# larskaislaniemi/PyLamp

Hardware: AMD Instinct MI355X
Metric: stokes_heat_mic_cell_updates_per_s (higher is better)
Workload: dtype f64

## Files before the change

pylamp_amd/csrc/pl_mic_cells.hip:

```cpp
#include "pl_internal.h"
#include "pl_mic.h"

#define SC_Q 4
#define SC_NL 16
#define SC_W (SC_NL - 2)
#ifndef SC_ROWS
#define SC_ROWS 32
#endif
#ifndef SC_CAP
#define SC_CAP 320
#endif
#define SC_CAPP (SC_CAP + SC_CAP / 16 + 2)
#ifndef SC_NB
#define SC_NB 2
#endif

__device__ inline int sc_pidx(int o) { return o + (o >> 4); }

template <int CTRL> __device__ inline double sc_dpp(double v) {
    int lo = __double2loint(v), hi = __double2hiint(v);
    lo = __builtin_amdgcn_update_dpp(0, lo, CTRL, 0xf, 0xf, false);
    hi = __builtin_amdgcn_update_dpp(0, hi, CTRL, 0xf, 0xf, false);
    return __hiloint2double(hi, lo);
}
__device__ inline double sc_left(double v) { return sc_dpp<0x111>(v); }
__device__ inline double sc_right(double v) { return sc_dpp<0x101>(v); }
__device__ inline double sc_qsum(double v) {
    unsigned lo = (unsigned)__double2loint(v), hi = (unsigned)__double2hiint(v);
    auto rl = __builtin_amdgcn_permlane16_swap(lo, lo, false, false);
    auto rh = __builtin_amdgcn_permlane16_swap(hi, hi, false, false);
    v = __hiloint2double((int)rh[0], (int)rl[0]) + __hiloint2double((int)rh[1], (int)rl[1]);
    lo = (unsigned)__double2loint(v); hi = (unsigned)__double2hiint(v);
    rl = __builtin_amdgcn_permlane32_swap(lo, lo, false, false);
    rh = __builtin_amdgcn_permlane32_swap(hi, hi, false, false);
    return __hiloint2double((int)rh[0], (int)rl[0]) + __hiloint2double((int)rh[1], (int)rl[1]);
}

template <int NFN, int CEN, bool MID>
struct ScAcc {
    double N[2][2][1 + NFN];
    double C[CEN ? 3 : 1][CEN ? 3 : 1][2];
    double Z[MID ? 3 : 1][MID ? 2 : 1][2];
    double X[MID ? 2 : 1][MID ? 3 : 1][2];
};

template <bool FLAT>
__device__ inline void sc_slots3(double a, double w[3]) {
    const bool lo = a < 0.5;
    if (FLAT) { w[0] = lo ? 1.0 : 0.0; w[1] = 1.0; w[2] = lo ? 0.0 : 1.0; }
    else { w[0] = lo ? 0.5 - a : 0.0; w[1] = lo ? a + 0.5 : 1.5 - a; w[2] = lo ? 0.0 : a - 0.5; }
}

#define SC_IND_MASK ((1u << 2) | (1u << 4) | (1u << 5))
template <int NFN, int CEN, bool MID, bool IND>
__global__ __launch_bounds__(64) void k_scatter_cells(PlScatterCellsArgs a, int strips_x) {
    constexpr int NST = 2 + NFN + (MID ? 1 : 0);
    constexpr unsigned IMASK = IND ? SC_IND_MASK : 0u;
    __shared__ double lds[NST][SC_CAPP];
    __shared__ int csl[SC_ROWS + 2][SC_NL + 1];
    const int lane = threadIdx.x, q = lane >> 4, L = lane & 15;
    const int sx = blockIdx.x % strips_x, sy = blockIdx.x / strips_x;
    const int c0 = sx * SC_W, r0 = sy * SC_ROWS, r1 = min(r0 + SC_ROWS, a.ncz);
    const int cc = c0 + L - 1;
    const bool real = cc >= 0 && cc < a.ncx;
    const int gj = a.ccol0 + cc;
    const int nown = min(SC_W, a.ncx - c0);
    const bool last_x = c0 + SC_W >= a.ncx, last_z = r1 >= a.ncz;
    const bool col_own = ((L >= 1 && L <= nown) || (sx == 0 && L == 0) || (last_x && L == nown + 1)) && gj >= 0 && gj < a.nx &&
                         gj >= a.col0 && gj < a.col0 + a.ncols;
    const int R0 = a.crow0 + (sy == 0 ? r0 - 1 : r0), R1 = a.crow0 + (last_z ? r1 + 1 : r1);
    const int i0 = max(r0 - 1, 0), i1 = min(r1 + 1, a.ncz);
    const int cfirst = max(c0 - 1, 0), clast = min(c0 + SC_W + 1, a.ncx);
    for (int k = lane; k < (i1 - i0) * (SC_NL + 1); k += 64) {
        const int r = k / (SC_NL + 1), c = k % (SC_NL + 1);
        const int col = min(max(c0 - 1 + c, cfirst), clast);
        csl[r][c] = a.cell_start[(long long)(i0 + r) * a.ncx + col];
    }
    const double xc = a.x0 + gj * a.hx;
    __shared__ double car[NFN + 11][SC_NL];
    double* const cN = &car[0][L];
    double* const cX = &car[NFN + 1][L]; double* const qZ = &car[NFN + 3][L]; double* const pZ = &car[NFN + 5][L];
    double* const qC = &car[NFN + 7][L]; double* const pC = &car[NFN + 9][L];
    if (q == 0)
        for (int k = 0; k < NFN + 11; k++) car[k][L] = 0.0;
    auto emit = [&](double* plane, int gi_row, double v) {
        if (!col_own || gi_row < R0 || gi_row >= R1 || gi_row < 0 || gi_row >= a.nz || gi_row < a.row0 || gi_row >= a.row0 + a.nrows) return;
        plane[(long long)(gi_row - a.row0) * a.ncols + (gj - a.col0)] = v;
    };
    __syncthreads();
    constexpr int NU = SC_CAP / 64;
    double pf[NU][NST];
    __shared__ int ixs[IND ? SC_CAP : 1];
    int pix[NU];
    auto prefetch = [&](int row) {
        const int b0 = csl[row - i0][0], b1 = min(b0 + SC_CAP, csl[row - i0][SC_NL]);
#pragma unroll
        for (int u = 0; u < NU; u++) {
            const int t = b0 + lane + 64 * u;
            if (t < b1) {
                pf[u][0] = a.tz[t]; pf[u][1] = a.tx[t];
                const int e = IND ? ixs[lane + 64 * u] : t;
#pragma unroll
                for (int k = 0; k < NFN; k++) pf[u][2 + k] = a.fn[k][(IMASK >> k) & 1u ? e : t];
                if (MID) pf[u][2 + NFN] = a.fm[IND ? e : t];
            }
        }
        if (IND && row + 1 < i1) {
            const int c0n = csl[row + 1 - i0][0], c1n = min(c0n + SC_CAP, csl[row + 1 - i0][SC_NL]);
#pragma unroll
            for (int u = 0; u < NU; u++) { const int t = c0n + lane + 64 * u; if (t < c1n) pix[u] = a.ix[t]; }
        }
    };
    if (i0 < i1 && !(a.dbg & 8)) {
        if (IND) {
            const int b0 = csl[0][0], b1 = min(b0 + SC_CAP, csl[0][SC_NL]);
#pragma unroll
            for (int u = 0; u < NU; u++) { const int t = b0 + lane + 64 * u; if (t < b1) ixs[lane + 64 * u] = a.ix[t]; }
            __syncthreads();
        }
        prefetch(i0);
    }
    for (int i = i0; i < i1; i++) {
        const int gi = a.crow0 + i;
        const double zc = a.z0 + gi * a.hz;
        const int wrow0 = csl[i - i0][0], wrow1 = csl[i - i0][SC_NL];
        int s = 0, e = 0;
        if (real) { s = csl[i - i0][L]; e = csl[i - i0][L + 1]; }
        ScAcc<NFN, CEN, MID> A;
#pragma unroll
        for (int di = 0; di < 2; di++)
#pragma unroll
            for (int dj = 0; dj < 2; dj++)
#pragma unroll
                for (int k = 0; k <= NFN; k++) A.N[di][dj][k] = 0.0;
        if (CEN) {
#pragma unroll
            for (int u = 0; u < 3; u++)
#pragma unroll
                for (int v = 0; v < 3; v++) { A.C[u][v][0] = 0.0; A.C[u][v][1] = 0.0; }
        }
        if (MID) {
#pragma unroll
            for (int u = 0; u < 3; u++)
#pragma unroll
                for (int v = 0; v < 2; v++) { A.Z[u][v][0] = 0.0; A.Z[u][v][1] = 0.0; A.X[v][u][0] = 0.0; A.X[v][u][1] = 0.0; }
        }
        if (!(a.dbg & 8)) {
            const int we0 = min(wrow0 + SC_CAP, wrow1);
#pragma unroll
            for (int u = 0; u < NU; u++) {
                const int t = wrow0 + lane + 64 * u;
                if (t < we0) {
                    const int o = sc_pidx(t - wrow0);
#pragma unroll
                    for (int k = 0; k < NST; k++) lds[k][o] = pf[u][k];
                }
            }
            if (IND && i + 1 < i1) {
                const int c0n = csl[i + 1 - i0][0], c1n = min(c0n + SC_CAP, csl[i + 1 - i0][SC_NL]);
#pragma unroll
                for (int u = 0; u < NU; u++) if (c0n + lane + 64 * u < c1n) ixs[lane + 64 * u] = pix[u];
            }
        }
        __syncthreads();
        if (i + 1 < i1 && !(a.dbg & 8)) prefetch(i + 1);
        for (int wb = wrow0; wb < wrow1; wb += SC_CAP) {
            const int we = min(wb + SC_CAP, wrow1);
            if (wb != wrow0) {
                __syncthreads();
                constexpr int UB = (NU + SC_NB - 1) / SC_NB;
#pragma unroll
                for (int b = 0; b < SC_NB; b++) {
                    double st[UB][NST];
#pragma unroll
                    for (int u = 0; u < UB; u++) {
                        const int t = wb + lane + 64 * (b * UB + u);
                        if (b * UB + u < NU && t < we) {
                            st[u][0] = a.tz[t]; st[u][1] = a.tx[t];
                            const int e = IND ? a.ix[t] : t;
#pragma unroll
                            for (int k = 0; k < NFN; k++) st[u][2 + k] = a.fn[k][(IMASK >> k) & 1u ? e : t];
                            if (MID) st[u][2 + NFN] = a.fm[IND ? e : t];
                        }
                    }
#pragma unroll
                    for (int u = 0; u < UB; u++) {
                        const int t = wb + lane + 64 * (b * UB + u);
                        if (b * UB + u < NU && t < we) {
                            const int o = sc_pidx(t - wb);
#pragma unroll
                            for (int k = 0; k < NST; k++) lds[k][o] = st[u][k];
                        }
                    }
                }
                __syncthreads();
            }
            int t = s + q;
            if (t < wb) t += ((wb - t + SC_Q - 1) / SC_Q) * SC_Q;
            const int tend = min(e, we);
            for (; t < tend && !(a.dbg & 1); t += SC_Q) {
                const int o = sc_pidx(t - wb);
                const double z = lds[0][o], x = lds[1][o];
                const double ca = (z - zc) * a.rhz, cb = (x - xc) * a.rhx;
                if (!(ca >= 0.0 && ca < 1.0 && cb >= 0.0 && cb < 1.0)) {
                    if (L >= 1 && L <= nown && i >= r0 && i < r1) {
                        const int k = atomicAdd(a.slow_count, 1);
                        if (k < a.slow_cap) a.slow_list[k] = t;
                    }
                    continue;
                }
                double f[NFN > 0 ? NFN : 1];
#pragma unroll
                for (int k = 0; k < NFN; k++) f[k] = lds[2 + k][o];
                const double wz2[2] = {1.0 - ca, ca}, wx2[2] = {1.0 - cb, cb};
#pragma unroll
                for (int di = 0; di < 2; di++)
#pragma unroll
                    for (int dj = 0; dj < 2; dj++) {
                        const double w = wx2[dj] * wz2[di];
                        A.N[di][dj][0] += w;
#pragma unroll
                        for (int k = 0; k < NFN; k++) A.N[di][dj][1 + k] += f[k] * w;
                    }
                double wz3[3], wx3[3];
                if (CEN || MID) { sc_slots3<CEN == 2>(ca, wz3); sc_slots3<CEN == 2>(cb, wx3); }
                if (CEN) {
                    const double fc = f[NFN > 1 ? 1 : 0];
#pragma unroll
                    for (int u = 0; u < 3; u++)
#pragma unroll
                        for (int v = 0; v < 3; v++) {
                            const double w = wx3[v] * wz3[u];
                            A.C[u][v][0] += w; A.C[u][v][1] += fc * w;
                        }
                }
                if (MID) {
                    const double fm = lds[2 + NFN][o];
#pragma unroll
                    for (int u = 0; u < 3; u++)
#pragma unroll
                        for (int v = 0; v < 2; v++) {
                            const double wzm = wx2[v] * wz3[u];
                            A.Z[u][v][0] += wzm; A.Z[u][v][1] += fm * wzm;
                            const double wxm = wx3[u] * wz2[v];
                            A.X[v][u][0] += wxm; A.X[v][u][1] += fm * wxm;
                        }
                }
            }
        }
        double Hn[2][1 + NFN], Hz[3][2], Hx[2][2], Hc[3][2];
#pragma unroll
        for (int di = 0; di < 2; di++)
#pragma unroll
            for (int k = 0; k <= NFN; k++) Hn[di][k] = sc_qsum(A.N[di][0][k] + sc_left(A.N[di][1][k]));
        if (MID) {
#pragma unroll
            for (int u = 0; u < 3; u++)
#pragma unroll
                for (int k = 0; k < 2; k++) Hz[u][k] = sc_qsum(A.Z[u][0][k] + sc_left(A.Z[u][1][k]));
#pragma unroll
            for (int v = 0; v < 2; v++)
#pragma unroll
                for (int k = 0; k < 2; k++) Hx[v][k] = sc_qsum(A.X[v][1][k] + sc_left(A.X[v][2][k]) + sc_right(A.X[v][0][k]));
        }
        if (CEN) {
#pragma unroll
            for (int u = 0; u < 3; u++)
#pragma unroll
                for (int k = 0; k < 2; k++) Hc[u][k] = sc_qsum(A.C[u][1][k] + sc_left(A.C[u][2][k]) + sc_right(A.C[u][0][k]));
        }
        if (q == 0 && !(a.dbg & 4)) {
#pragma unroll
            for (int k = 0; k <= NFN; k++) {
                emit(a.accN + (long long)k * a.N, gi, Hn[0][k] + cN[k * SC_NL]);
                cN[k * SC_NL] = Hn[1][k];
            }
            if (MID) {
#pragma unroll
                for (int k = 0; k < 2; k++) {
                    emit(a.accX + (long long)k * a.N, gi, Hx[0][k] + cX[k * SC_NL]);
                    cX[k * SC_NL] = Hx[1][k];
                    emit(a.accZ + (long long)k * a.N, gi - 1, qZ[k * SC_NL] + Hz[0][k]);
                    qZ[k * SC_NL] = Hz[1][k] + pZ[k * SC_NL]; pZ[k * SC_NL] = Hz[2][k];
                }
            }
            if (CEN) {
#pragma unroll
                for (int k = 0; k < 2; k++) {
                    emit(a.accC + (long long)k * a.N, gi - 1, qC[k * SC_NL] + Hc[0][k]);
                    qC[k * SC_NL] = Hc[1][k] + pC[k * SC_NL]; pC[k * SC_NL] = Hc[2][k];
                }
            }
        }
        __syncthreads();
    }
    if (q == 0 && i1 > i0 && !(a.dbg & 4)) {
        const int gl = a.crow0 + i1;
#pragma unroll
        for (int k = 0; k <= NFN; k++) emit(a.accN + (long long)k * a.N, gl, cN[k * SC_NL]);
        if (MID) {
#pragma unroll
            for (int k = 0; k < 2; k++) {
                emit(a.accX + (long long)k * a.N, gl, cX[k * SC_NL]);
                emit(a.accZ + (long long)k * a.N, gl - 1, qZ[k * SC_NL]);
                emit(a.accZ + (long long)k * a.N, gl, pZ[k * SC_NL]);
            }
        }
        if (CEN) {
#pragma unroll
            for (int k = 0; k < 2; k++) {
                emit(a.accC + (long long)k * a.N, gl - 1, qC[k * SC_NL]);
                emit(a.accC + (long long)k * a.N, gl, pC[k * SC_NL]);
            }
        }
    }
}

template <int NFN, int CEN, bool MID, bool IND>
__global__ __launch_bounds__(256) void k_scatter_cells_slow(PlScatterCellsArgs a) {
    constexpr unsigned IMASK = IND ? SC_IND_MASK : 0u;
    const int n = min(*a.slow_count, a.slow_cap);
    for (int k = blockIdx.x * 256 + threadIdx.x; k < n; k += gridDim.x * 256) {
        const int t = a.slow_list[k];
        const int e = IND ? a.ix[t] : t;
        const double z = a.tz[t], x = a.tx[t];
        auto add = [&](double* plane, int ni, int nj, double v) {
            if (ni < 0 || ni >= a.nz || nj < 0 || nj >= a.nx || ni < a.row0 || ni >= a.row0 + a.nrows || nj < a.col0 || nj >= a.col0 + a.ncols) return;
            unsafeAtomicAdd(plane + (long long)(ni - a.row0) * a.ncols + (nj - a.col0), v);
        };
        for (int set = 0; set < 4; set++) {
            if ((set == 1 && !CEN) || (set >= 2 && !MID)) continue;
            const bool sz = set == 1 || set == 2, sx = set == 1 || set == 3;
            const double zo = a.z0 + (sz ? 0.5 * a.hz : 0.0), xo = a.x0 + (sx ? 0.5 * a.hx : 0.0);
            const double fz = floor((z - zo) * a.rhz), fx = floor((x - xo) * a.rhx);
            const int ie = (int)fz, je = (int)fx;
            const double ca = (z - (zo + fz * a.hz)) * a.rhz, cb = (x - (xo + fx * a.hx)) * a.rhx;
            double* base = set == 0 ? a.accN : set == 1 ? a.accC : set == 2 ? a.accZ : a.accX;
            const int nfs = set == 0 ? NFN : 1;
            for (int cnr = 0; cnr < 4; cnr++) {
                const int di = cnr & 1, dj = cnr >> 1;
                double w = (dj ? cb : 1.0 - cb) * (di ? ca : 1.0 - ca);
                const bool flat = set == 1 && CEN == 2;
                if (flat) w = 1.0;
                add(base, ie + di, je + dj, w);
                for (int f = 0; f < nfs; f++) {
                    const int fk = set == 0 ? f : (NFN > 1 ? 1 : 0);
                    const double v = set <= 1 ? a.fn[fk][(IMASK >> fk) & 1u ? e : t] : a.fm[IND ? e : t];
                    add(base + (long long)(1 + f) * a.N, ie + di, je + dj, v * w);
                }
            }
        }
    }
}

__global__ __launch_bounds__(256) void k_scatter_finalize_multi(PlScatterFinalArgs a) {
    const int j = blockIdx.x * 64 + threadIdx.x, i = blockIdx.y * 4 + threadIdx.y;
    if (j >= a.nx || i >= a.nz) return;
    const long long o = (long long)i * a.acc_pitch + j, oo = a.out_off + (long long)i * a.out_pitch + j;
    for (int k = 0; k < a.nf; k++) {
        double s = a.acc[k][o];
        const double d = a.den[k][o];
        double r;
        if (a.scheme[k] & PL_AVG_ARITHMETIC) r = s / d;
        else { if (isinf(s)) s = 0.0; r = exp(s / d); }
        a.out[k][oo] = r;
    }
}

void pl_launch_scatter_finalize_multi(pl_ctx* ctx, const PlScatterFinalArgs& a) {
    if (a.nf <= 0) return;
    hipLaunchKernelGGL(k_scatter_finalize_multi, dim3((a.nx + 63) / 64, (a.nz + 3) / 4), dim3(64, 4), 0, ctx->stream, a);
}

template <int NFN, int CEN, bool MID, bool IND = false>
static void launch_cells(pl_ctx* ctx, const PlScatterCellsArgs& a) {
    const int strips_x = (a.ncx + SC_W - 1) / SC_W, strips_z = (a.ncz + SC_ROWS - 1) / SC_ROWS;
    hipLaunchKernelGGL((k_scatter_cells<NFN, CEN, MID, IND>), dim3((unsigned)(strips_x * strips_z)), dim3(64), 0, ctx->stream, a, strips_x);
    hipLaunchKernelGGL((k_scatter_cells_slow<NFN, CEN, MID, IND>), dim3(32), dim3(256), 0, ctx->stream, a);
}

int pl_scatter_cells_device(pl_ctx* ctx, PlScatterCellsArgs& a, int variant) {
    if (a.ncz <= 0 || a.ncx <= 0) return 0;
    a.rhz = 1.0 / a.hz; a.rhx = 1.0 / a.hx;
    PL_HIP(ctx, hipMemsetAsync(a.slow_count, 0, sizeof(int), ctx->stream));
    if (a.ix && (variant != 0 || a.ind != (SC_IND_MASK | (1u << 31)))) return pl_fail(ctx, "pl_scatter_cells_device: unsupported set of indexed fields");
    if (variant == 0 && a.ix) launch_cells<6, 1, true, true>(ctx, a);
    else if (variant == 0) launch_cells<6, 1, true>(ctx, a);
    else if (variant == 1) launch_cells<2, 2, false>(ctx, a);
    else if (variant == 2) launch_cells<1, 0, false>(ctx, a);
    else return pl_fail(ctx, "pl_scatter_cells_device: unknown variant");
    PL_HIP(ctx, hipGetLastError());
    return 0;
}
```

Baseline: 203.3 million.

## Split scatter accumulator sets across waves and add deterministic listed slow path

The per-strip marker-to-grid scatter kernel now runs several wavefronts per block, each owning a subset of the accumulator sets (nodal, centre, z-mid, x-mid). The wavefronts share the staged LDS marker data and split the prefetch/copy work. This lowers per-wave register pressure and raises parallelism per strip, at the cost of redundant weight computation and larger blocks. A new single-block kernel handles up to 2048 out-of-cell markers without atomics, using a rank sort and row-banded serial accumulation. It is launched every call, even when there are no such markers, which adds launch latency.

Measured after the change: 206.3 million (median of 6 runs). 1.01x the previous value.

```diff
diff --git a/pylamp_amd/csrc/pl_mic_cells.hip b/pylamp_amd/csrc/pl_mic_cells.hip
--- a/pylamp_amd/csrc/pl_mic_cells.hip
+++ b/pylamp_amd/csrc/pl_mic_cells.hip
@@ -36,12 +36,25 @@
     return __hiloint2double((int)rh[0], (int)rl[0]) + __hiloint2double((int)rh[1], (int)rl[1]);
 }
 
-template <int NFN, int CEN, bool MID>
+#define SC_SET_N 1u
+#define SC_SET_C 2u
+#define SC_SET_Z 4u
+#define SC_SET_X 8u
+constexpr int sc_split_nw(int split) { return split == 1 ? 4 : split == 2 ? 3 : split == 3 ? 2 : 1; }
+constexpr unsigned sc_split_sets(int split, int w) {
+    return split == 1 ? (1u << w) : split == 2 ? (w == 0 ? SC_SET_N : w == 1 ? SC_SET_C : (SC_SET_Z | SC_SET_X))
+         : split == 3 ? (w == 0 ? SC_SET_N : (SC_SET_C | SC_SET_Z | SC_SET_X)) : (SC_SET_N | SC_SET_C | SC_SET_Z | SC_SET_X);
+}
+#ifndef SC_SPLIT_HEAT
+#define SC_SPLIT_HEAT 2
+#endif
+
+template <int NFN, bool SN, int CEN, bool SZ, bool SX>
 struct ScAcc {
-    double N[2][2][1 + NFN];
+    double N[SN ? 2 : 1][SN ? 2 : 1][SN ? 1 + NFN : 1];
     double C[CEN ? 3 : 1][CEN ? 3 : 1][2];
-    double Z[MID ? 3 : 1][MID ? 2 : 1][2];
-    double X[MID ? 2 : 1][MID ? 3 : 1][2];
+    double Z[SZ ? 3 : 1][SZ ? 2 : 1][2];
+    double X[SX ? 2 : 1][SX ? 3 : 1][2];
 };
 
 template <bool FLAT>
@@ -52,13 +65,15 @@
 }
 
 #define SC_IND_MASK ((1u << 2) | (1u << 4) | (1u << 5))
-template <int NFN, int CEN, bool MID, bool IND>
-__global__ __launch_bounds__(64) void k_scatter_cells(PlScatterCellsArgs a, int strips_x) {
+template <int NFN, int CEN, bool MID, bool IND, int NW, unsigned SETS>
+__device__ __forceinline__ void sc_strip(const PlScatterCellsArgs a, int strips_x, double (&lds)[2 + NFN + (MID ? 1 : 0)][SC_CAPP],
+                                         int (&csl)[SC_ROWS + 2][SC_NL + 1], double (&car)[NFN + 11][SC_NL], int (&ixs)[IND ? SC_CAP : 1]) {
     constexpr int NST = 2 + NFN + (MID ? 1 : 0);
     constexpr unsigned IMASK = IND ? SC_IND_MASK : 0u;
-    __shared__ double lds[NST][SC_CAPP];
-    __shared__ int csl[SC_ROWS + 2][SC_NL + 1];
-    const int lane = threadIdx.x, q = lane >> 4, L = lane & 15;
+    constexpr int NT = 64 * NW;
+    constexpr bool SN = (SETS & SC_SET_N) != 0, SC = (SETS & SC_SET_C) != 0 && CEN != 0, SZ = (SETS & SC_SET_Z) != 0 && MID,
+                   SX = (SETS & SC_SET_X) != 0 && MID;
+    const int tid = threadIdx.x, lane = tid & 63, q = lane >> 4, L = lane & 15;
     const int sx = blockIdx.x % strips_x, sy = blockIdx.x / strips_x;
     const int c0 = sx * SC_W, r0 = sy * SC_ROWS, r1 = min(r0 + SC_ROWS, a.ncz);
     const int cc = c0 + L - 1;
@@ -71,35 +86,33 @@
     const int R0 = a.crow0 + (sy == 0 ? r0 - 1 : r0), R1 = a.crow0 + (last_z ? r1 + 1 : r1);
     const int i0 = max(r0 - 1, 0), i1 = min(r1 + 1, a.ncz);
     const int cfirst = max(c0 - 1, 0), clast = min(c0 + SC_W + 1, a.ncx);
-    for (int k = lane; k < (i1 - i0) * (SC_NL + 1); k += 64) {
+    for (int k = tid; k < (i1 - i0) * (SC_NL + 1); k += NT) {
         const int r = k / (SC_NL + 1), c = k % (SC_NL + 1);
         const int col = min(max(c0 - 1 + c, cfirst), clast);
         csl[r][c] = a.cell_start[(long long)(i0 + r) * a.ncx + col];
     }
     const double xc = a.x0 + gj * a.hx;
-    __shared__ double car[NFN + 11][SC_NL];
     double* const cN = &car[0][L];
     double* const cX = &car[NFN + 1][L]; double* const qZ = &car[NFN + 3][L]; double* const pZ = &car[NFN + 5][L];
     double* const qC = &car[NFN + 7][L]; double* const pC = &car[NFN + 9][L];
-    if (q == 0)
+    if (tid < SC_NL)
         for (int k = 0; k < NFN + 11; k++) car[k][L] = 0.0;
     auto emit = [&](double* plane, int gi_row, double v) {
         if (!col_own || gi_row < R0 || gi_row >= R1 || gi_row < 0 || gi_row >= a.nz || gi_row < a.row0 || gi_row >= a.row0 + a.nrows) return;
         plane[(long long)(gi_row - a.row0) * a.ncols + (gj - a.col0)] = v;
     };
     __syncthreads();
-    constexpr int NU = SC_CAP / 64;
+    constexpr int NU = (SC_CAP + NT - 1) / NT;
     double pf[NU][NST];
-    __shared__ int ixs[IND ? SC_CAP : 1];
     int pix[NU];
     auto prefetch = [&](int row) {
         const int b0 = csl[row - i0][0], b1 = min(b0 + SC_CAP, csl[row - i0][SC_NL]);
 #pragma unroll
         for (int u = 0; u < NU; u++) {
-            const int t = b0 + lane + 64 * u;
+            const int t = b0 + tid + NT * u;
             if (t < b1) {
                 pf[u][0] = a.tz[t]; pf[u][1] = a.tx[t];
-                const int e = IND ? ixs[lane + 64 * u] : t;
+                const int e = IND ? ixs[tid + NT * u] : t;
 #pragma unroll
                 for (int k = 0; k < NFN; k++) pf[u][2 + k] = a.fn[k][(IMASK >> k) & 1u ? e : t];
                 if (MID) pf[u][2 + NFN] = a.fm[IND ? e : t];
@@ -108,14 +121,14 @@
         if (IND && row + 1 < i1) {
             const int c0n = csl[row + 1 - i0][0], c1n = min(c0n + SC_CAP, csl[row + 1 - i0][SC_NL]);
 #pragma unroll
-            for (int u = 0; u < NU; u++) { const int t = c0n + lane + 64 * u; if (t < c1n) pix[u] = a.ix[t]; }
+            for (int u = 0; u < NU; u++) { const int t = c0n + tid + NT * u; if (t < c1n) pix[u] = a.ix[t]; }
         }
     };
     if (i0 < i1 && !(a.dbg & 8)) {
         if (IND) {
             const int b0 = csl[0][0], b1 = min(b0 + SC_CAP, csl[0][SC_NL]);
 #pragma unroll
-            for (int u = 0; u < NU; u++) { const int t = b0 + lane + 64 * u; if (t < b1) ixs[lane + 64 * u] = a.ix[t]; }
+            for (int u = 0; u < NU; u++) { const int t = b0 + tid + NT * u; if (t < b1) ixs[tid + NT * u] = a.ix[t]; }
             __syncthreads();
         }
         prefetch(i0);
@@ -126,30 +139,33 @@
         const int wrow0 = csl[i - i0][0], wrow1 = csl[i - i0][SC_NL];
         int s = 0, e = 0;
         if (real) { s = csl[i - i0][L]; e = csl[i - i0][L + 1]; }
-        ScAcc<NFN, CEN, MID> A;
-#pragma unroll
-        for (int di = 0; di < 2; di++)
-#pragma unroll
-            for (int dj = 0; dj < 2; dj++)
-#pragma unroll
-                for (int k = 0; k <= NFN; k++) A.N[di][dj][k] = 0.0;
-        if (CEN) {
+        ScAcc<NFN, SN, SC ? CEN : 0, SZ, SX> A;
+        if constexpr (SN) {
+#pragma unroll
+            for (int di = 0; di < 2; di++)
+#pragma unroll
+                for (int dj = 0; dj < 2; dj++)
+#pragma unroll
+                    for (int k = 0; k <= NFN; k++) A.N[di][dj][k] = 0.0;
+        }
+        if constexpr (SC) {
 #pragma unroll
             for (int u = 0; u < 3; u++)
 #pragma unroll
                 for (int v = 0; v < 3; v++) { A.C[u][v][0] = 0.0; A.C[u][v][1] = 0.0; }
         }
-        if (MID) {
-#pragma unroll
-            for (int u = 0; u < 3; u++)
-#pragma unroll
-                for (int v = 0; v < 2; v++) { A.Z[u][v][0] = 0.0; A.Z[u][v][1] = 0.0; A.X[v][u][0] = 0.0; A.X[v][u][1] = 0.0; }
-        }
+#pragma unroll
+        for (int u = 0; u < 3; u++)
+#pragma unroll
+            for (int v = 0; v < 2; v++) {
+                if constexpr (SZ) { A.Z[u][v][0] = 0.0; A.Z[u][v][1] = 0.0; }
+                if constexpr (SX) { A.X[v][u][0] = 0.0; A.X[v][u][1] = 0.0; }
+            }
         if (!(a.dbg & 8)) {
             const int we0 = min(wrow0 + SC_CAP, wrow1);
 #pragma unroll
             for (int u = 0; u < NU; u++) {
-                const int t = wrow0 + lane + 64 * u;
+                const int t = wrow0 + tid + NT * u;
                 if (t < we0) {
                     const int o = sc_pidx(t - wrow0);
 #pragma unroll
@@ -159,7 +175,7 @@
             if (IND && i + 1 < i1) {
                 const int c0n = csl[i + 1 - i0][0], c1n = min(c0n + SC_CAP, csl[i + 1 - i0][SC_NL]);
 #pragma unroll
-                for (int u = 0; u < NU; u++) if (c0n + lane + 64 * u < c1n) ixs[lane + 64 * u] = pix[u];
+                for (int u = 0; u < NU; u++) if (c0n + tid + NT * u < c1n) ixs[tid + NT * u] = pix[u];
             }
         }
         __syncthreads();
@@ -174,18 +190,18 @@
                     double st[UB][NST];
 #pragma unroll
                     for (int u = 0; u < UB; u++) {
-                        const int t = wb + lane + 64 * (b * UB + u);
+                        const int t = wb + tid + NT * (b * UB + u);
                         if (b * UB + u < NU && t < we) {
                             st[u][0] = a.tz[t]; st[u][1] = a.tx[t];
                             const int e = IND ? a.ix[t] : t;
 #pragma unroll
                             for (int k = 0; k < NFN; k++) st[u][2 + k] = a.fn[k][(IMASK >> k) & 1u ? e : t];
-                            if (MID) st[u][2 + NFN] = a.fm[IND ? e : t];
+                            if constexpr (MID) st[u][2 + NFN] = a.fm[IND ? e : t];
                         }
                     }
 #pragma unroll
                     for (int u = 0; u < UB; u++) {
-                        const int t = wb + lane + 64 * (b * UB + u);
+                        const int t = wb + tid + NT * (b * UB + u);
                         if (b * UB + u < NU && t < we) {
                             const int o = sc_pidx(t - wb);
 #pragma unroll
@@ -203,29 +219,31 @@
                 const double z = lds[0][o], x = lds[1][o];
                 const double ca = (z - zc) * a.rhz, cb = (x - xc) * a.rhx;
                 if (!(ca >= 0.0 && ca < 1.0 && cb >= 0.0 && cb < 1.0)) {
-                    if (L >= 1 && L <= nown && i >= r0 && i < r1) {
+                    if (SN && L >= 1 && L <= nown && i >= r0 && i < r1) {
                         const int k = atomicAdd(a.slow_count, 1);
                         if (k < a.slow_cap) a.slow_list[k] = t;
                     }
                     continue;
                 }
+                const double wz2[2] = {1.0 - ca, ca}, wx2[2] = {1.0 - cb, cb};
                 double f[NFN > 0 ? NFN : 1];
-#pragma unroll
-                for (int k = 0; k < NFN; k++) f[k] = lds[2 + k][o];
-                const double wz2[2] = {1.0 - ca, ca}, wx2[2] = {1.0 - cb, cb};
-#pragma unroll
-                for (int di = 0; di < 2; di++)
-#pragma unroll
-                    for (int dj = 0; dj < 2; dj++) {
-                        const double w = wx2[dj] * wz2[di];
-                        A.N[di][dj][0] += w;
-#pragma unroll
-                        for (int k = 0; k < NFN; k++) A.N[di][dj][1 + k] += f[k] * w;
-                    }
+                if constexpr (SN) {
+#pragma unroll
+                    for (int k = 0; k < NFN; k++) f[k] = lds[2 + k][o];
+#pragma unroll
+                    for (int di = 0; di < 2; di++)
+#pragma unroll
+                        for (int dj = 0; dj < 2; dj++) {
+                            const double w = wx2[dj] * wz2[di];
+                            A.N[di][dj][0] += w;
+#pragma unroll
+                            for (int k = 0; k < NFN; k++) A.N[di][dj][1 + k] += f[k] * w;
+                        }
+                }
                 double wz3[3], wx3[3];
-                if (CEN || MID) { sc_slots3<CEN == 2>(ca, wz3); sc_slots3<CEN == 2>(cb, wx3); }
-                if (CEN) {
-                    const double fc = f[NFN > 1 ? 1 : 0];
+                if constexpr (SC || SZ || SX) { sc_slots3<CEN == 2>(ca, wz3); sc_slots3<CEN == 2>(cb, wx3); }
+                if constexpr (SC) {
+                    const double fc = SN ? f[NFN > 1 ? 1 : 0] : lds[2 + (NFN > 1 ? 1 : 0)][o];
 #pragma unroll
                     for (int u = 0; u < 3; u++)
 #pragma unroll
@@ -234,57 +252,69 @@
                             A.C[u][v][0] += w; A.C[u][v][1] += fc * w;
                         }
                 }
-                if (MID) {
+                if constexpr (SZ || SX) {
                     const double fm = lds[2 + NFN][o];
 #pragma unroll
                     for (int u = 0; u < 3; u++)
 #pragma unroll
                         for (int v = 0; v < 2; v++) {
-                            const double wzm = wx2[v] * wz3[u];
-                            A.Z[u][v][0] += wzm; A.Z[u][v][1] += fm * wzm;
-                            const double wxm = wx3[u] * wz2[v];
-                            A.X[v][u][0] += wxm; A.X[v][u][1] += fm * wxm;
+                            if constexpr (SZ) {
+                                const double wzm = wx2[v] * wz3[u];
+                                A.Z[u][v][0] += wzm; A.Z[u][v][1] += fm * wzm;
+                            }
+                            if constexpr (SX) {
+                                const double wxm = wx3[u] * wz2[v];
+                                A.X[v][u][0] += wxm; A.X[v][u][1] += fm * wxm;
+                            }
                         }
                 }
             }
         }
         double Hn[2][1 + NFN], Hz[3][2], Hx[2][2], Hc[3][2];
-#pragma unroll
-        for (int di = 0; di < 2; di++)
-#pragma unroll
-            for (int k = 0; k <= NFN; k++) Hn[di][k] = sc_qsum(A.N[di][0][k] + sc_left(A.N[di][1][k]));
-        if (MID) {
+        if constexpr (SN) {
+#pragma unroll
+            for (int di = 0; di < 2; di++)
+#pragma unroll
+                for (int k = 0; k <= NFN; k++) Hn[di][k] = sc_qsum(A.N[di][0][k] + sc_left(A.N[di][1][k]));
+        }
+        if constexpr (SZ) {
 #pragma unroll
             for (int u = 0; u < 3; u++)
 #pragma unroll
                 for (int k = 0; k < 2; k++) Hz[u][k] = sc_qsum(A.Z[u][0][k] + sc_left(A.Z[u][1][k]));
+        }
+        if constexpr (SX) {
 #pragma unroll
             for (int v = 0; v < 2; v++)
 #pragma unroll
                 for (int k = 0; k < 2; k++) Hx[v][k] = sc_qsum(A.X[v][1][k] + sc_left(A.X[v][2][k]) + sc_right(A.X[v][0][k]));
         }
-        if (CEN) {
+        if constexpr (SC) {
 #pragma unroll
             for (int u = 0; u < 3; u++)
 #pragma unroll
                 for (int k = 0; k < 2; k++) Hc[u][k] = sc_qsum(A.C[u][1][k] + sc_left(A.C[u][2][k]) + sc_right(A.C[u][0][k]));
         }
         if (q == 0 && !(a.dbg & 4)) {
-#pragma unroll
-            for (int k = 0; k <= NFN; k++) {
-                emit(a.accN + (long long)k * a.N, gi, Hn[0][k] + cN[k * SC_NL]);
-                cN[k * SC_NL] = Hn[1][k];
-            }
-            if (MID) {
-#pragma unroll
-                for (int k = 0; k < 2; k++) {
+            if constexpr (SN) {
+#pragma unroll
+                for (int k = 0; k <= NFN; k++) {
+                    emit(a.accN + (long long)k * a.N, gi, Hn[0][k] + cN[k * SC_NL]);
+                    cN[k * SC_NL] = Hn[1][k];
+                }
+            }
+#pragma unroll
+            for (int k = 0; k < 2; k++) {
+                if constexpr (SX) {
                     emit(a.accX + (long long)k * a.N, gi, Hx[0][k] + cX[k * SC_NL]);
                     cX[k * SC_NL] = Hx[1][k];
+                }
+                if constexpr (SZ) {
                     emit(a.accZ + (long long)k * a.N, gi - 1, qZ[k * SC_NL] + Hz[0][k]);
                     qZ[k * SC_NL] = Hz[1][k] + pZ[k * SC_NL]; pZ[k * SC_NL] = Hz[2][k];
                 }
             }
-            if (CEN) {
+            if constexpr (SC) {
 #pragma unroll
                 for (int k = 0; k < 2; k++) {
                     emit(a.accC + (long long)k * a.N, gi - 1, qC[k * SC_NL] + Hc[0][k]);
@@ -296,22 +326,96 @@
     }
     if (q == 0 && i1 > i0 && !(a.dbg & 4)) {
         const int gl = a.crow0 + i1;
-#pragma unroll
-        for (int k = 0; k <= NFN; k++) emit(a.accN + (long long)k * a.N, gl, cN[k * SC_NL]);
-        if (MID) {
-#pragma unroll
-            for (int k = 0; k < 2; k++) {
-                emit(a.accX + (long long)k * a.N, gl, cX[k * SC_NL]);
+        if constexpr (SN) {
+#pragma unroll
+            for (int k = 0; k <= NFN; k++) emit(a.accN + (long long)k * a.N, gl, cN[k * SC_NL]);
+        }
+#pragma unroll
+        for (int k = 0; k < 2; k++) {
+            if constexpr (SX) emit(a.accX + (long long)k * a.N, gl, cX[k * SC_NL]);
+            if constexpr (SZ) {
                 emit(a.accZ + (long long)k * a.N, gl - 1, qZ[k * SC_NL]);
                 emit(a.accZ + (long long)k * a.N, gl, pZ[k * SC_NL]);
             }
         }
-        if (CEN) {
+        if constexpr (SC) {
 #pragma unroll
             for (int k = 0; k < 2; k++) {
                 emit(a.accC + (long long)k * a.N, gl - 1, qC[k * SC_NL]);
                 emit(a.accC + (long long)k * a.N, gl, pC[k * SC_NL]);
             }
+        }
+    }
+}
+
+template <int NFN, int CEN, bool MID, bool IND, int SPLIT>
+__global__ __launch_bounds__(64 * sc_split_nw(SPLIT)) void k_scatter_cells(PlScatterCellsArgs a, int strips_x) {
+    constexpr int NW = sc_split_nw(SPLIT);
+    __shared__ double lds[2 + NFN + (MID ? 1 : 0)][SC_CAPP];
+    __shared__ int csl[SC_ROWS + 2][SC_NL + 1];
+    __shared__ double car[NFN + 11][SC_NL];
+    __shared__ int ixs[IND ? SC_CAP : 1];
+    const int wv = NW > 1 ? __builtin_amdgcn_readfirstlane((int)threadIdx.x >> 6) : 0;
+    if (wv == 0) sc_strip<NFN, CEN, MID, IND, NW, sc_split_sets(SPLIT, 0)>(a, strips_x, lds, csl, car, ixs);
+    if constexpr (NW > 1) { if (wv == 1) sc_strip<NFN, CEN, MID, IND, NW, sc_split_sets(SPLIT, 1)>(a, strips_x, lds, csl, car, ixs); }
+    if constexpr (NW > 2) { if (wv == 2) sc_strip<NFN, CEN, MID, IND, NW, sc_split_sets(SPLIT, 2)>(a, strips_x, lds, csl, car, ixs); }
+    if constexpr (NW > 3) { if (wv == 3) sc_strip<NFN, CEN, MID, IND, NW, sc_split_sets(SPLIT, 3)>(a, strips_x, lds, csl, car, ixs); }
+}
+
+#define SC_SLOW_DET 2048
+#define SC_SLOW_BANDS 64
+template <int NFN, int CEN, bool MID, bool IND>
+__global__ __launch_bounds__(1024) void k_scatter_cells_listed(PlScatterCellsArgs a) {
+    constexpr unsigned IMASK = IND ? SC_IND_MASK : 0u;
+    constexpr int NPL = (1 + NFN) + (CEN ? 2 : 0) + (MID ? 4 : 0);
+    static_assert(NPL * SC_SLOW_BANDS <= 1024, "one thread per plane and band");
+    __shared__ int raw[SC_SLOW_DET], srt[SC_SLOW_DET];
+    const int n = min(*a.slow_count, a.slow_cap);
+    if (n <= 0 || n > SC_SLOW_DET) return;
+    const int tid = threadIdx.x;
+    for (int k = tid; k < n; k += 1024) raw[k] = a.slow_list[k];
+    __syncthreads();
+    for (int k = tid; k < n; k += 1024) {
+        const int v = raw[k];
+        int r = 0;
+        for (int j = 0; j < n; j++) r += (raw[j] < v || (raw[j] == v && j < k)) ? 1 : 0;
+        srt[r] = v;
+    }
+    __syncthreads();
+    const int p = tid / SC_SLOW_BANDS, band = tid % SC_SLOW_BANDS;
+    if (p >= NPL) return;
+    int set = 0, k = p;
+    if (k >= 1 + NFN) { k -= 1 + NFN; set = CEN ? 1 : 2; if (CEN && k >= 2) { k -= 2; set = 2; } if (set == 2 && k >= 2) { k -= 2; set = 3; } }
+    const bool sz = set == 1 || set == 2, sx = set == 1 || set == 3;
+    const double zo = a.z0 + (sz ? 0.5 * a.hz : 0.0), xo = a.x0 + (sx ? 0.5 * a.hx : 0.0);
+    double* const plane = (set == 0 ? a.accN : set == 1 ? a.accC : set == 2 ? a.accZ : a.accX) + (long long)k * a.N;
+    const bool flat = set == 1 && CEN == 2;
+    const int fk = set == 0 ? k - 1 : (NFN > 1 ? 1 : 0);
+    for (int q = 0; q < n; q++) {
+        const int t = srt[q];
+        const double fz = floor((a.tz[t] - zo) * a.rhz);
+        const int ie = (int)fz;
+        const bool row0 = ((ie % SC_SLOW_BANDS) + SC_SLOW_BANDS) % SC_SLOW_BANDS == band;
+        const bool row1 = (((ie + 1) % SC_SLOW_BANDS) + SC_SLOW_BANDS) % SC_SLOW_BANDS == band;
+        if (!row0 && !row1) continue;
+        const double z = a.tz[t], x = a.tx[t];
+        const double fx = floor((x - xo) * a.rhx);
+        const int je = (int)fx;
+        const double ca = (z - (zo + fz * a.hz)) * a.rhz, cb = (x - (xo + fx * a.hx)) * a.rhx;
+        double v = 1.0;
+        if (k > 0) {
+            const int e = IND ? a.ix[t] : t;
+            v = set <= 1 ? a.fn[fk][(IMASK >> fk) & 1u ? e : t] : a.fm[IND ? e : t];
+        }
+        for (int cnr = 0; cnr < 4; cnr++) {
+            const int di = cnr & 1, dj = cnr >> 1;
+            if (!(di ? row1 : row0)) continue;
+            const int ni = ie + di, nj = je + dj;
+            if (ni < 0 || ni >= a.nz || nj < 0 || nj >= a.nx || ni < a.row0 || ni >= a.row0 + a.nrows || nj < a.col0 || nj >= a.col0 + a.ncols) continue;
+            double w = (dj ? cb : 1.0 - cb) * (di ? ca : 1.0 - ca);
+            if (flat) w = 1.0;
+            double* const dst = plane + (long long)(ni - a.row0) * a.ncols + (nj - a.col0);
+            *dst = __dadd_rn(*dst, k > 0 ? __dmul_rn(v, w) : w);
         }
     }
 }
@@ -320,6 +424,7 @@
 __global__ __launch_bounds__(256) void k_scatter_cells_slow(PlScatterCellsArgs a) {
     constexpr unsigned IMASK = IND ? SC_IND_MASK : 0u;
     const int n = min(*a.slow_count, a.slow_cap);
+    if (n <= SC_SLOW_DET) return;
     for (int k = blockIdx.x * 256 + threadIdx.x; k < n; k += gridDim.x * 256) {
         const int t = a.slow_list[k];
         const int e = IND ? a.ix[t] : t;
@@ -372,10 +477,17 @@
     hipLaunchKernelGGL(k_scatter_finalize_multi, dim3((a.nx + 63) / 64, (a.nz + 3) / 4), dim3(64, 4), 0, ctx->stream, a);
 }
 
-template <int NFN, int CEN, bool MID, bool IND = false>
+static bool sc_split_on() { const char* e = getenv("PYLAMP_SC_SPLIT"); return !(e && atoi(e) == 0); }
+
+template <int NFN, int CEN, bool MID, bool IND, int SPLIT>
 static void launch_cells(pl_ctx* ctx, const PlScatterCellsArgs& a) {
     const int strips_x = (a.ncx + SC_W - 1) / SC_W, strips_z = (a.ncz + SC_ROWS - 1) / SC_ROWS;
-    hipLaunchKernelGGL((k_scatter_cells<NFN, CEN, MID, IND>), dim3((unsigned)(strips_x * strips_z)), dim3(64), 0, ctx->stream, a, strips_x);
+    const dim3 grid((unsigned)(strips_x * strips_z));
+    if (SPLIT != 0 && sc_split_on())
+        hipLaunchKernelGGL((k_scatter_cells<NFN, CEN, MID, IND, SPLIT>), grid, dim3(64 * sc_split_nw(SPLIT)), 0, ctx->stream, a, strips_x);
+    else
+        hipLaunchKernelGGL((k_scatter_cells<NFN, CEN, MID, IND, 0>), grid, dim3(64), 0, ctx->stream, a, strips_x);
+    hipLaunchKernelGGL((k_scatter_cells_listed<NFN, CEN, MID, IND>), dim3(1), dim3(1024), 0, ctx->stream, a);
     hipLaunchKernelGGL((k_scatter_cells_slow<NFN, CEN, MID, IND>), dim3(32), dim3(256), 0, ctx->stream, a);
 }
 
@@ -384,10 +496,10 @@
     a.rhz = 1.0 / a.hz; a.rhx = 1.0 / a.hx;
     PL_HIP(ctx, hipMemsetAsync(a.slow_count, 0, sizeof(int), ctx->stream));
     if (a.ix && (variant != 0 || a.ind != (SC_IND_MASK | (1u << 31)))) return pl_fail(ctx, "pl_scatter_cells_device: unsupported set of indexed fields");
-    if (variant == 0 && a.ix) launch_cells<6, 1, true, true>(ctx, a);
-    else if (variant == 0) launch_cells<6, 1, true>(ctx, a);
-    else if (variant == 1) launch_cells<2, 2, false>(ctx, a);
-    else if (variant == 2) launch_cells<1, 0, false>(ctx, a);
+    if (variant == 0 && a.ix) launch_cells<6, 1, true, true, SC_SPLIT_HEAT>(ctx, a);
+    else if (variant == 0) launch_cells<6, 1, true, false, SC_SPLIT_HEAT>(ctx, a);
+    else if (variant == 1) launch_cells<2, 2, false, false, 3>(ctx, a);
+    else if (variant == 2) launch_cells<1, 0, false, false, 0>(ctx, a);
     else return pl_fail(ctx, "pl_scatter_cells_device: unknown variant");
     PL_HIP(ctx, hipGetLastError());
     return 0;
```
